# gildas-lormeau/zlib-streams-ts

Measured on AMD Instinct MI355X. Metric: uncompressed MB/s, deflate-raw L6, 4096x64KiB batch at 1/2/4/8 GPUs, higher is better.
Workload: dtype u8; 1 GPU; 4096 x 65536 B text-corpus streams split across the GPUs, deflate-raw level 6; global_streams=4096, streams_per_gpu=4096, stream_bytes=65536, level=6, format=deflate-raw, compressed_bytes=91855591, parallelism=dp1

## Files before the change

zlib-streams-ts_amd/csrc/capi.cpp:

```cpp
#include <hip/hip_runtime.h>
#include <stdint.h>
#include <stdio.h>
#include <string.h>

#include <algorithm>
#include <string>
#include <thread>
#include <vector>

#include "../../include/zs_gpu.h"
#include "zs_common.h"
#include "zs_kernels.h"
#include "zs_inflate.h"
#include "zs_split.h"
#include "zs_seg.h"
#include "zs_plan.h"
#include "zs_sweep_ring.h"
#include "zs_dict.h"


namespace {

thread_local std::string g_err;

// ... 958 lines not shown
  const zs_meta_layout ml(n);
  Batch b;
  const int r = upload_batch(c, st, ml, ml.bytes + (seeds ? 4ull * n : 0), {n, d_in, in_off, in_len, nullptr, nullptr, nullptr},
                             &b, [&](uint8_t* hm) { if (seeds) memcpy(hm + ml.bytes, seeds, 4ull * n); });
  if (r != ZS_OK) return r;
  MARK("start");
  zs_k_checksum<<<n, 64, 0, st>>>(b.in, b.in_off, b.in_len, d_check, kind,
                                  seeds ? (const uint32_t*)(c->meta.as<uint8_t>() + ml.bytes) : nullptr);
  MARK("checksum");
  HIPCHK(hipGetLastError());
  return ZS_OK;
}

extern "C" int zs_crc32_batch_device(zs_ctx* c, uint32_t n, const uint8_t* d_in, const uint64_t* in_off,
                                     const uint32_t* in_len, const uint32_t* seeds, uint32_t* d_check,
                                     void* hip_stream) {
  return checksum_batch(c, 2, n, d_in, in_off, in_len, seeds, d_check, hip_stream);
}
extern "C" int zs_adler32_batch_device(zs_ctx* c, uint32_t n, const uint8_t* d_in, const uint64_t* in_off,
                                       const uint32_t* in_len, const uint32_t* seeds, uint32_t* d_check,
                                       void* hip_stream) {
  return checksum_batch(c, 1, n, d_in, in_off, in_len, seeds, d_check, hip_stream);
}

static int checksum_host(zs_ctx* c, int kind, uint32_t n, const uint8_t* in, const uint64_t* in_off,
                         const uint32_t* in_len, const uint32_t* seeds, uint32_t* check) {
  if (!c) return fail(ZS_STREAM_ERROR, "null context");
  HIPCHK(hipSetDevice(c->device));
  if (n == 0) return ZS_OK;
  std::vector<uint64_t> doff;
  uint64_t total = 0;
  int r = stage_in(c, n, in, in_off, in_len, doff, total);
  if (r != ZS_OK) return r;
  HIPCHK(c->d_res.ensure(4ull * n + 16));
  r = checksum_batch(c, kind, n, c->d_in.as<uint8_t>(), doff.data(), in_len, seeds, c->d_res.as<uint32_t>(), nullptr);
  if (r != ZS_OK) return r;
  HIPCHK(hipMemcpyAsync(check, c->d_res.p, 4ull * n, hipMemcpyDeviceToHost, c->stream));
  HIPCHK(hipStreamSynchronize(c->stream));
  return ZS_OK;
}
extern "C" int zs_crc32_batch(zs_ctx* c, uint32_t n, const uint8_t* in, const uint64_t* in_off,
                              const uint32_t* in_len, const uint32_t* seeds, uint32_t* check) {
  return checksum_host(c, 2, n, in, in_off, in_len, seeds, check);
}
extern "C" int zs_adler32_batch(zs_ctx* c, uint32_t n, const uint8_t* in, const uint64_t* in_off,
                                const uint32_t* in_len, const uint32_t* seeds, uint32_t* check) {
  return checksum_host(c, 1, n, in, in_off, in_len, seeds, check);
}

namespace {
const char* kVocab =
    "the of and to in is that for it as was with be by on not he this are or his from at which but have an they you "
    "were her she there been one all we their has would when if so no will more can out said up what about its into "
    "them than only other new some could time these two may then do first any my now such like our over man me even "
    "most made after also did many before must through back years where much your way well down should because each "
    "just those people how too little state good very make world still own see men work long get here between both "
    "life being under never day same another know while last might us great old year off come since against go came "
    "right used take three";

struct XS {
  uint32_t s;
  explicit XS(uint32_t seed) : s(seed ? seed : 1) {}
  uint32_t operator()() {
    s ^= s << 13;
    s ^= s >> 17;
    s ^= s << 5;
    return s;
  }
};

void gen_text(uint32_t seed, uint8_t* out, uint32_t n, const std::vector<std::string>& V) {
  XS r(seed);
  uint32_t o = 0, w = 0;
  while (o < n) {
    const uint32_t a = r();
    const uint32_t idx = std::min(a % 144u, (a >> 12) % 144u);
    const std::string& word = V[idx];
    for (size_t i = 0; i < word.size() && o < n; i++) out[o++] = (uint8_t)word[i];
    if (o < n) out[o++] = (++w % 13 == 0) ? 10 : 32;
  }
}
}

extern "C" void zs_corpus(int kind, uint32_t first, uint32_t n_streams, uint32_t len, uint8_t* out, int threads) {
  std::vector<std::string> V;
  {
    std::string all(kVocab), cur;
    for (char ch : all) {
      if (ch == ' ') { V.push_back(cur); cur.clear(); }
      else cur.push_back(ch);
    }
    V.push_back(cur);
  }
  auto one = [&](uint32_t i) {
    const uint32_t seed = 0x9e3779b9u ^ (first + i);
    uint8_t* o = out + (size_t)i * len;
    if (kind == 2) {
      XS r(seed);
      for (uint32_t j = 0; j < len; j++) o[j] = (uint8_t)r();
      return;
    }
    gen_text(seed, o, len, V);
    if (kind == 1) {
      XS r(seed ^ 0x85ebca6bu);
      for (uint32_t k = 0; k + 8192 <= len; k += 8192)
        for (uint32_t j = 0; j < 1024; j++) o[k + 4096 + j] = (uint8_t)r();
    }
  };
  if (threads < 1) threads = 1;
  std::vector<std::thread> th;
  for (int t = 0; t < threads; t++)
    th.emplace_back([&, t] {
      for (uint32_t i = (uint32_t)t; i < n_streams; i += (uint32_t)threads) one(i);
    });
  for (auto& x : th) x.join();
}

extern "C" uint64_t zs_debug_fetch(zs_ctx* c, int what, uint32_t s, void* dst, uint64_t cap) {
  if (c && what >= 16 && what <= 21) {
    (void)hipSetDevice(c->device);
    (void)hipDeviceSynchronize();
    const Buf* b = what == 16 ? &c->gcnt : what == 17 ? &c->gblk : what == 18 ? &c->glanes : what == 19 ? &c->gmem
                   : what == 21 ? &c->gent : &c->gfound;
    const uint64_t bytes = std::min<uint64_t>(cap, b->cap);
    if (!b->p || !bytes || hipMemcpy(dst, b->p, bytes, hipMemcpyDeviceToHost) != hipSuccess) return 0;
    return bytes;
  }
  if (!c || !c->streams.p) return 0;
  (void)hipSetDevice(c->device);
  (void)hipStreamSynchronize(c->stream);
  (void)hipDeviceSynchronize();
  zs_stream st;
  if (hipMemcpy(&st, c->streams.as<zs_stream>() + s, sizeof st, hipMemcpyDeviceToHost) != hipSuccess) return 0;
  uint64_t pos_base = 0;
  uint32_t blk_base = 0, n = 0;
  const size_t nstreams = c->last_n;
  zs_meta_layout m2((uint32_t)nstreams);
  const uint8_t* hm = c->hmeta.data();
  pos_base = ((const uint64_t*)(hm + m2.pos_base))[s];
  blk_base = ((const uint32_t*)(hm + m2.blk_base))[s];
  n = ((const uint32_t*)(hm + m2.in_len))[s];
  if (s < c->dp.start.size()) n += c->dp.start[s];
  const void* src = nullptr;
  uint64_t bytes = 0;
  if ((what == 0 && 2ull * (pos_base + n) > c->prevd.cap) || (what == 1 && 8ull * (pos_base + n) > c->mres.cap)) return 0;
  switch (what) {
    case 0: src = c->prevd.as<uint16_t>() + pos_base; bytes = 2ull * n; break;
    case 1: src = c->mres.as<uint2>() + pos_base; bytes = 8ull * n; break;
    case 2: src = c->syms.as<uint32_t>() + pos_base + s; bytes = 4ull * st.nsym; break;
    case 3: src = c->blocks.as<zs_block>() + blk_base; bytes = sizeof(zs_block) * st.nblk; break;
    case 4: src = c->streams.as<zs_stream>() + s; bytes = sizeof(zs_stream); break;
    case 5: src = c->codes.as<uint32_t>() + (size_t)blk_base * (ZS_L_CODES + ZS_D_CODES); bytes = 4ull * (ZS_L_CODES + ZS_D_CODES) * st.nblk; break;
    case 6: src = c->hdr.as<uint32_t>() + (size_t)blk_base * ZS_HDR_WORDS; bytes = 4ull * ZS_HDR_WORDS * st.nblk; break;
    default: return 0;
  }
  bytes = std::min(bytes, cap);
  if (bytes && hipMemcpy(dst, src, bytes, hipMemcpyDeviceToHost) != hipSuccess) return 0;
  return bytes;
}

static const char* kInflateMsgs[ZS_MSG_COUNT] = {
    "",
    "incorrect header check",
    "unknown compression method",
    "invalid window size",
    "unknown header flags set",
    "header crc mismatch",
    "invalid block type",
    "invalid stored block lengths",
    "too many length or distance symbols",
    "too many length",
    "invalid code lengths set",
    "invalid bit length repeat",
    "invalid code -- missing end-of-block",
    "invalid literal/lengths set",
    "invalid distances set",
    "invalid literal/length code",
    "invalid distance code",
    "invalid distance too far back",
    "incorrect data check",
    "incorrect length check",
    "output capacity exceeded",
};

extern "C" const char* zs_inflate_message(int32_t i) { return (i >= 0 && i < ZS_MSG_COUNT) ? kInflateMsgs[i] : ""; }

__global__ void zs_k_inflate_finish(const zs_inflate_result* r, const zs_lane_res* lane, int32_t* status,
                                    int32_t* phase, int32_t* msg, uint32_t* out_len, uint32_t* consumed, int n,
                                    uint32_t* lane_count) {
  const int s = blockIdx.x * blockDim.x + threadIdx.x;
  if (s >= n) return;
  if (lane && lane[s].bail == 0) {
    atomicAdd(lane_count, 1u);
    status[s] = ZS_Z_STREAM_END;
    phase[s] = ZS_PHASE_NONE_;
    msg[s] = ZS_MSG_NONE;
    out_len[s] = lane[s].out_len;
    consumed[s] = lane[s].consumed;
    return;
  }
  status[s] = r[s].status;
  phase[s] = r[s].phase;
  msg[s] = r[s].msg;
  out_len[s] = r[s].out_len;
  consumed[s] = r[s].consumed;
}

__global__ void zs_k_inflate_check(const uint8_t* in, const uint64_t* in_off, const int32_t* status,
                                   const uint32_t* consumed, int wbits, uint32_t* out, int n) {
  const int s = blockIdx.x * blockDim.x + threadIdx.x;
  if (s >= n) return;
  uint32_t v = 0;
  if (status[s] == ZS_Z_STREAM_END && wbits > 0) {
    const uint8_t* t = in + in_off[s] + consumed[s] - (wbits == 31 ? 8 : 4);
    v = wbits == 31 ? (uint32_t)t[0] | (uint32_t)t[1] << 8 | (uint32_t)t[2] << 16 | (uint32_t)t[3] << 24
                    : (uint32_t)t[0] << 24 | (uint32_t)t[1] << 16 | (uint32_t)t[2] << 8 | (uint32_t)t[3];
  }
  out[s] = v;
}

static auto lane_kernel(int rt, bool refw) {
  return refw ? (rt == 2 ? zs_k_inflate_lane<2, true> : zs_k_inflate_lane<0, true>)
              : (rt == 2   ? zs_k_inflate_lane<2, false>
                 : rt == 1 ? zs_k_inflate_lane<1, false>
                           : zs_k_inflate_lane<0, false>);
}
static auto lane_kernel_dict(int rt) {
  return rt == 2 ? zs_k_inflate_lane<2, false, true> : rt == 1 ? zs_k_inflate_lane<1, false, true>
                                                               : zs_k_inflate_lane<0, false, true>;
}

static int seg_launch(zs_ctx* c, hipStream_t st, int wbits, const Batch& h, const Batch& b, zs_lane_res* lres) {
  const std::vector<uint32_t>& list = c->ip.seg;
  zs_seg_plan& p = c->gp;
  zs_plan_seg(c->o, wbits, list, h.in_len, h.out_cap, p);
  const uint32_t ng = (uint32_t)list.size(), nb = p.nb, nbig = (uint32_t)p.big.size();
  HIPCHK(c->glist.ensure(4ull * ng));
  HIPCHK(c->gspb.ensure(4ull * (ng + 1)));
  HIPCHK(c->gbig.ensure(4ull * nbig + 4));
  HIPCHK(c->gfound.ensure(8ull * ZS_SPLIT_MAX * nbig + 8));
  HIPCHK(c->gblk.ensure(sizeof(zs_seg_blk) * nb));
  HIPCHK(c->glanes.ensure(sizeof(zs_seg_lane) * ZS_SEG_LANES * nb));
  HIPCHK(c->gtab.ensure(sizeof(zcode) * ZS_SEG_TAB * nb));
  HIPCHK(c->gent.ensure(sizeof(zs_seg_ent) * ZS_SPLIT_MAX * ng));
  HIPCHK(c->gmem.ensure(sizeof(zs_seg_mem) * ng));
  HIPCHK(c->gpbase.ensure(4ull * (ng + 1)));
  HIPCHK(c->gplist.ensure(16ull * p.pbase[ng] + 16));
  HIPCHK(c->gsbase.ensure(8ull * (ng + 1)));
  HIPCHK(c->gscr.ensure(2ull * p.sbase[ng] + 64));
  HIPCHK(c->gcnt.ensure(16));
  HIPCHK(c->gspl.ensure(4ull * nb + 4));
  HIPCHK(c->gflist.ensure(4ull * ng));
  if (nbig) HIPCHK(c->gbigs.ensure(4ull * nbig));
  HIPCHK(hipMemcpyAsync(c->glist.p, list.data(), 4ull * ng, hipMemcpyHostToDevice, st));
  HIPCHK(hipMemcpyAsync(c->gspb.p, p.spb.data(), 4ull * (ng + 1), hipMemcpyHostToDevice, st));
  HIPCHK(hipMemcpyAsync(c->gpbase.p, p.pbase.data(), 4ull * (ng + 1), hipMemcpyHostToDevice, st));
  HIPCHK(hipMemcpyAsync(c->gsbase.p, p.sbase.data(), 8ull * (ng + 1), hipMemcpyHostToDevice, st));
  if (nbig) {
    HIPCHK(hipMemcpyAsync(c->gbigs.p, p.big_s.data(), 4ull * nbig, hipMemcpyHostToDevice, st));
    HIPCHK(hipMemcpyAsync(c->gbig.p, p.big.data(), 4ull * nbig, hipMemcpyHostToDevice, st));
  }
  HIPCHK(hipMemsetAsync(c->gmem.p, 0, sizeof(zs_seg_mem) * ng, st));
  HIPCHK(hipMemsetAsync(c->gent.p, 0, sizeof(zs_seg_ent) * ZS_SPLIT_MAX * ng, st));
  HIPCHK(hipMemsetAsync(c->gblk.p, 0xff, sizeof(zs_seg_blk) * nb, st));
  HIPCHK(hipMemsetAsync(c->gcnt.as<uint32_t>() + 2, 0, 8, st));
  if (!c->keep_counts) HIPCHK(hipMemsetAsync(c->gcnt.p, 0, 8, st));
  HIPCHK(hipEventRecord(c->fork, st));
  HIPCHK(hipStreamWaitEvent(c->side, c->fork, 0));
  hipStream_t sd = c->side;
  if (int r = mark(c, sd, "start")) return r;
  const uint32_t* gl = c->glist.as<uint32_t>();
  uint64_t* gf = c->gfound.as<uint64_t>();
  uint32_t* cnt = c->gcnt.as<uint32_t>();
  zs_seg_blk* gb = c->gblk.as<zs_seg_blk>();
  zs_seg_lane* gln = c->glanes.as<zs_seg_lane>();
  zcode* gt = c->gtab.as<zcode>();
  zs_seg_ent* ge = c->gent.as<zs_seg_ent>();
  zs_seg_mem* gm = c->gmem.as<zs_seg_mem>();
  const uint32_t* spl = c->gspl.as<uint32_t>();
  const uint64_t* sb = c->gsbase.as<uint64_t>();
  uint16_t* scr = c->gscr.as<uint16_t>();
  uint32_t* llen = c->llen.as<uint32_t>();
  if (nbig) {
    zs_k_split_find<<<nbig * ZS_SPLIT_MAX, 256, 0, sd>>>(b.in, b.in_off, b.in_len, c->gbigs.as<uint32_t>(), wbits, gf);
    if (int r = mark(c, sd, "seg_find")) return r;
  }
  auto walk = p.d64 ? (p.w2k ? zs_k_seg_walk<true, 2048u, false> : zs_k_seg_walk<true, 1024u, false>)
                    : (p.w2k ? zs_k_seg_walk<false, 2048u, true>
                             : p.large ? zs_k_seg_walk<false, 1024u, true> : zs_k_seg_walk<false, 1024u, false>);
  walk<<<p.nwalk, 64, 0, sd>>>(b.in, b.in_off, b.in_len, gl, ng, c->gbig.as<uint32_t>(), nbig, wbits, gf,
                               c->gspb.as<uint32_t>(), gb, gln, gt, ge, gm, cnt + 2, c->gspl.as<uint32_t>(), p.walk_bits,
                               p.split);
  if (int r = mark(c, sd, "seg_walk")) return r;
  zs_k_seg_plan<<<ng, 64, 0, sd>>>(b.in, b.in_off, b.in_len, b.out_cap, gl, ng, wbits, p.refw ? 1 : 0, gb, gln, ge, gm,
                                   c->gpbase.as<uint32_t>(), c->gplist.as<uint4>());
  if (int r = mark(c, sd, "seg_plan")) return r;
  auto decode = p.d64 ? zs_k_seg_decode<true, false> : p.refw ? zs_k_seg_decode<false, true> : zs_k_seg_decode<false, false>;
  decode<<<p.gdec, 64, 0, sd>>>(b.in, b.in_off, b.in_len, gl, cnt + 2, spl, gb, gln, gt, gm, sb, scr);
  if (int r = mark(c, sd, "seg_decode")) return r;
  const int rsm = p.rsmall ? 65536 : 32768;
  auto resolve = p.rsmall ? zs_k_seg_resolve<512u, 65536u> : zs_k_seg_resolve<256u, 32768u>;
  HIPCHK(hipFuncSetAttribute((const void*)resolve, hipFuncAttributeMaxDynamicSharedMemorySize, rsm));
  resolve<<<ng, p.rsmall ? 512u : 256u, rsm, sd>>>(gl, gm, c->gpbase.as<uint32_t>(), c->gplist.as<uint4>(), sb, scr, b.out,
                                             b.out_off, lres, llen, cnt + 1, cnt + 3, c->gflist.as<uint32_t>());
  if (int r = mark(c, sd, "seg_resolve")) return r;
  const size_t wsm = zs_inflate_wave_lds_bytes(p.d64);
// ... 292 lines not shown
```

zlib-streams-ts_amd/csrc/deflate_sweep.hip:

```cpp
#include <hip/hip_runtime.h>
#include "zs_common.h"
#include "zs_kernels.h"
#include "zs_sweep_ring.h"
#include "zs_sweep_long.h"
#include "zs_sweep_ends.h"
#include <type_traits>
#include <utility>

#define ZS_SW_WIN_WORDS ((ZS_SEG_WPOS + 258u + 20u + 3u) / 4u + 2u)
#define ZS_SW_RING 128u
#define ZS_SW_MW 320u
#ifndef ZS_SW_RUN_CAP
#define ZS_SW_RUN_CAP 16u
#endif

typedef __attribute__((address_space(3))) uint32_t zs_sw_lds_u32;
static __device__ __forceinline__ uint32_t sw_lds_addr(const void* p) {
  return (uint32_t)(uintptr_t)(const zs_sw_lds_u32*)p;
}

static __device__ __forceinline__ uint32_t sw_hash(uint32_t w) {
  return (((w & 0xffu) << 10) ^ (((w >> 8) & 0xffu) << 5) ^ ((w >> 16) & 0xffu)) & ZS_HASH_MASK;
}

#define ZS_BK_WPT (16384u / ZS_BK_THREADS)
#define ZS_BK_PPL (ZS_BK_THREADS / 64u)
#ifndef ZS_BK_PROF
#define ZS_BK_PROF 0
#endif
#if ZS_BK_PROF
__device__ unsigned long long zs_bk_stat[4];
extern "C" int zs_bucket_stats(unsigned long long* out) {
  return (int)hipMemcpyFromSymbol(out, HIP_SYMBOL(zs_bk_stat), sizeof(zs_bk_stat));
}
#define BK_MARK(i) do { if (threadIdx.x == 0) { const unsigned long long t_ = wall_clock64(); atomicAdd(&zs_bk_stat[i], t_ - bk_t); bk_t = t_; } } while (0)
#else
#define BK_MARK(i) do { } while (0)
#endif
#define ZS_BK_INFLIGHT 8
#define ZS_BK_CHUNK 2048u

template <bool ORD>
__global__ __launch_bounds__(ZS_BK_THREADS) void zs_k_bucket(const uint8_t* __restrict__ in,
                                                            const uint64_t* __restrict__ in_off,
                                                            const uint32_t* __restrict__ in_len,
                                                            const uint64_t* __restrict__ pos_base,
                                                            const zs_sweep_seg* __restrict__ segs,
                                                            uint16_t* __restrict__ members, uint2* __restrict__ mres) {
  __shared__ uint32_t cnt[16384];
  __shared__ uint32_t part[ZS_BK_THREADS];
  __shared__ uint32_t stg[ZS_BK_CHUNK / 4 + 2];
  __shared__ uint16_t q[2][ZS_BK_CHUNK];
  const zs_sweep_seg G = segs[blockIdx.x];
  const int s = (int)G.s;
  const uint32_t nrel = in_len[s] - G.base;
  const uint32_t tid = threadIdx.x;
  const uint8_t* src = in + in_off[s] + G.base;
  uint16_t* mem = members + G.mb;
  uint2* out = mres + pos_base[s] + G.base;
  const uint32_t m = nrel > 2 ? min(nrel - 2, G.ohi) : 0u;
  const uint32_t n = min(nrel, m + 2u);
  if (nrel - m <= 2u)
    for (uint32_t p = m + tid; p < nrel; p += ZS_BK_THREADS) out[p] = make_uint2(0, 0);
  if (m == 0) return;
  for (uint32_t i = tid; i < 16384 / 4; i += ZS_BK_THREADS) reinterpret_cast<uint4*>(cnt)[i] = make_uint4(0, 0, 0, 0);
  const bool aligned = ((uintptr_t)src & 3u) == 0;
#if ZS_BK_PROF
  unsigned long long bk_t = wall_clock64();
  if (threadIdx.x == 0) atomicAdd(&zs_bk_stat[3], 1ull);
#endif
  __syncthreads();
  {
    uint32_t w[5], nw[5];
    auto load5 = [&](uint32_t p0, uint32_t* x) __attribute__((always_inline)) {
#pragma unroll
      for (int k = 0; k < 5; k++) x[k] = zs_load_word(src, n, p0 + 16 * tid + 4 * k);
    };
    load5(0, nw);
    for (uint32_t p0 = 0; p0 < m; p0 += 16 * ZS_BK_THREADS) {
#pragma unroll
      for (int k = 0; k < 5; k++) w[k] = nw[k];
      if (p0 + 16 * ZS_BK_THREADS < m) load5(p0 + 16 * ZS_BK_THREADS, nw);
#pragma unroll
      for (uint32_t j = 0; j < 16; j++) {
        const uint32_t p = p0 + 16 * tid + j;
        const uint32_t h = sw_hash(__builtin_amdgcn_alignbyte(w[(j >> 2) + 1], w[j >> 2], j & 3u));
        if (p < m) atomicAdd(&cnt[h >> 1], 1u << (16u * (h & 1u)));
      }
    }
  }
  __syncthreads();
  BK_MARK(0);
  {
    uint32_t sum = 0;
    for (uint32_t j = 0; j < ZS_BK_WPT; j++) {
      const uint32_t w = cnt[ZS_BK_WPT * tid + ((j + tid) & (ZS_BK_WPT - 1u))];
      sum += (w & 0xffffu) + (w >> 16);
    }
    part[tid] = sum;
    __syncthreads();
    if (tid < 64) {
      uint32_t v[ZS_BK_PPL], t = 0;
#pragma unroll
      for (uint32_t j = 0; j < ZS_BK_PPL; j++) { v[j] = part[ZS_BK_PPL * tid + j]; t += v[j]; }
      uint32_t x = t;
#pragma unroll
      for (int d = 1; d < 64; d <<= 1) {
        const uint32_t y = __shfl_up(x, d, 64);
        if (tid >= (uint32_t)d) x += y;
      }
      uint32_t run = x - t;
#pragma unroll
      for (uint32_t j = 0; j < ZS_BK_PPL; j++) { part[ZS_BK_PPL * tid + j] = run; run += v[j]; }
    }
    __syncthreads();
    uint32_t run = part[tid];
    for (uint32_t j = 0; j < ZS_BK_WPT; j++) {
      const uint32_t w = cnt[ZS_BK_WPT * tid + j];
      const uint32_t lo = w & 0xffffu;
      cnt[ZS_BK_WPT * tid + j] = run | ((run + lo) << 16);
      run += lo + (w >> 16);
    }
  }
  __syncthreads();
  BK_MARK(1);
  const uint32_t wave = tid >> 6, lane = tid & 63u;
  constexpr uint32_t CW = ZS_BK_CHUNK / 4 / 64;
  uint32_t nxt[CW + 1];
  auto fetch = [&](uint32_t c0) {
#pragma unroll
    for (uint32_t i = 0; i <= CW; i++) {
      const uint32_t w = 64 * i + lane;
      const uint32_t at = c0 + 4 * w;
      uint32_t v = 0;
      if (w < ZS_BK_CHUNK / 4 + 2) {
        if (aligned && at + 4 <= n) v = *(const uint32_t*)(src + at);
        else
          for (uint32_t k = 0; k < 4; k++)
            if (at + k < n) v |= (uint32_t)src[at + k] << (8 * k);
      }
      nxt[i] = v;
    }
  };
  if (wave == 0) fetch(0);
  const uint32_t nch = (m + ZS_BK_CHUNK - 1) / ZS_BK_CHUNK;
  for (uint32_t c = 0; c <= nch; c++) {
    const uint32_t c0 = c * ZS_BK_CHUNK;
    if (wave == 0 && c < nch) {
      __builtin_amdgcn_s_waitcnt(0xc07f);
      __builtin_amdgcn_wave_barrier();
#pragma unroll
      for (uint32_t i = 0; i <= CW; i++)
        if (64 * i + lane < ZS_BK_CHUNK / 4 + 2) stg[64 * i + lane] = nxt[i];
      __builtin_amdgcn_s_waitcnt(0xc07f);
      __builtin_amdgcn_wave_barrier();
      if (c0 + ZS_BK_CHUNK < m) fetch(c0 + ZS_BK_CHUNK);
      const uint32_t c1 = min(m, c0 + ZS_BK_CHUNK);
      uint16_t* const qc = q[c & 1u];
      for (uint32_t g0 = c0; g0 < c1; g0 += 64 * ZS_BK_INFLIGHT) {
        uint32_t a[ZS_BK_INFLIGHT], v[ZS_BK_INFLIGHT], sh[ZS_BK_INFLIGHT], e[ZS_BK_INFLIGHT], hh[ZS_BK_INFLIGHT];
#pragma unroll
        for (int j = 0; j < ZS_BK_INFLIGHT; j++) {
          const uint32_t p = g0 + 64 * j + lane;
          const uint32_t o = p - c0;
          const uint32_t h = sw_hash(__builtin_amdgcn_alignbyte(stg[(o >> 2) + 1], stg[o >> 2], o & 3u));
          hh[j] = h;
          sh[j] = 16u * (h & 1u);
          a[j] = sw_lds_addr(&cnt[h >> 1]);
          v[j] = p < c1 ? 1u << sh[j] : 0u;
        }
        if (!ORD) {
#pragma unroll
          for (int j = 0; j < ZS_BK_INFLIGHT; j++) {
            const uint32_t p = g0 + 64 * j + lane;
            const uint32_t h = hh[j];
            const uint64_t mm = zs_wave_match(h, p < c1);
            const uint32_t rank = (uint32_t)__builtin_popcountll(mm & ((1ull << lane) - 1ull));
            const uint32_t lead = mm ? (uint32_t)__builtin_ctzll(mm) : lane;
            uint32_t old = 0;
            if (p < c1 && lead == lane)
              old = atomicAdd(&cnt[h >> 1], (uint32_t)__builtin_popcountll(mm) << sh[j]);
            old = (uint32_t)__builtin_amdgcn_ds_bpermute((int)(lead * 4u), (int)old);
            e[j] = old + (rank << sh[j]);
          }
        } else {
        asm volatile(
            "ds_add_rtn_u32 %0, %8, %16\n\t"
            "ds_add_rtn_u32 %1, %9, %17\n\t"
            "ds_add_rtn_u32 %2, %10, %18\n\t"
            "ds_add_rtn_u32 %3, %11, %19\n\t"
            "ds_add_rtn_u32 %4, %12, %20\n\t"
            "ds_add_rtn_u32 %5, %13, %21\n\t"
            "ds_add_rtn_u32 %6, %14, %22\n\t"
            "ds_add_rtn_u32 %7, %15, %23\n\t"
            "s_waitcnt lgkmcnt(0)"
            : "=&v"(e[0]), "=&v"(e[1]), "=&v"(e[2]), "=&v"(e[3]), "=&v"(e[4]), "=&v"(e[5]), "=&v"(e[6]), "=&v"(e[7])
            : "v"(a[0]), "v"(a[1]), "v"(a[2]), "v"(a[3]), "v"(a[4]), "v"(a[5]), "v"(a[6]), "v"(a[7]), "v"(v[0]),
              "v"(v[1]), "v"(v[2]), "v"(v[3]), "v"(v[4]), "v"(v[5]), "v"(v[6]), "v"(v[7])
            : "memory");
        }
#pragma unroll
        for (int j = 0; j < ZS_BK_INFLIGHT; j++) {
          const uint32_t p = g0 + 64 * j + lane;
          if (p < c1) qc[p - c0] = (uint16_t)(e[j] >> sh[j]);
        }
      }
    } else if (wave != 0 && c > 0) {
      const uint32_t b0 = c0 - ZS_BK_CHUNK, cnt1 = min(m, c0) - b0;
      const uint16_t* const qp = q[(c - 1) & 1u];
      for (uint32_t o = tid - 64u; o < cnt1; o += ZS_BK_THREADS - 64u) mem[qp[o]] = (uint16_t)(b0 + o);
    }
    __syncthreads();
  }
  BK_MARK(2);
}
template __global__ void zs_k_bucket<true>(const uint8_t*, const uint64_t*, const uint32_t*, const uint64_t*,
                                           const zs_sweep_seg*, uint16_t*, uint2*);
template __global__ void zs_k_bucket<false>(const uint8_t*, const uint64_t*, const uint32_t*, const uint64_t*,
                                            const zs_sweep_seg*, uint16_t*, uint2*);

static __device__ __forceinline__ uint32_t sw_word(const uint32_t* win, uint32_t off) {
  const uint32_t i = off >> 2;
  return __builtin_amdgcn_alignbyte(win[i + 1], win[i], off & 3u);
}

static __device__ __forceinline__ uint32_t sw_extend(const uint32_t* win, uint32_t p, uint32_t q, uint32_t maxc,
                                                     uint32_t from) {
  uint32_t k = from;
  while (k < maxc) {
    const uint32_t y = sw_word(win, q + k) ^ sw_word(win, p + k);
    if (y) { k += (uint32_t)(__builtin_ctz(y) >> 3); break; }
    k += 4;
  }
  return k < maxc ? k : maxc;
}

static __device__ __forceinline__ uint32_t max3(uint32_t a, uint32_t b, uint32_t c) {
  return max(max(a, b), c);
}

static __device__ __forceinline__ uint32_t sw_x7(uint32_t w) {
  const uint32_t b0 = w & 0xffu, b1 = (w >> 8) & 0xffu;
  return ((b0 >> 5) & 3u) | ((b1 & 7u) << 2) | (((b1 >> 5) & 3u) << 5);
}
template <bool A7>
struct SwSig;
template <>
struct SwSig<false> {
  static constexpr uint32_t LONG = 88u;
  static constexpr uint32_t THR0 = 23u;
  static constexpr uint32_t EXT = 11u;
  uint32_t a, b, c;
  static __device__ __forceinline__ uint4 rec(const uint32_t* win, uint32_t q, uint32_t w0) {
    return make_uint4(w0, sw_word(win, q + 4), sw_word(win, q + 8) & 0x00ffffffu, 0u);
  }
  __device__ __forceinline__ uint32_t mbits(uint32_t x, uint32_t y, uint32_t z) const {
    uint32_t f0, f1, f2;
    asm("v_ffbl_b32 %0, %1" : "=v"(f0) : "v"(x ^ a));
    asm("v_ffbl_b32 %0, %1\n\tv_add_u32_e64 %0, %0, 32 clamp" : "=&v"(f1) : "v"(y ^ b));
    asm("v_ffbl_b32 %0, %1\n\tv_add_u32_e32 %0, 64, %0" : "=&v"(f2) : "v"(z ^ c));
    return min(min(f0, f1), f2);
  }
  template <uint32_t U>
  __device__ __forceinline__ uint32_t step(uint32_t x, uint32_t y, uint32_t z) const {
    return (mbits(x, y, z) & ~7u) | (7u - U);
  }
  template <uint32_t U>
  __device__ __forceinline__ uint32_t step(uint32_t x, uint32_t y, uint32_t z, uint64_t lm) const {
    uint32_t r;
    asm("v_cndmask_b32_e64 %0, 0, %1, %2" : "=v"(r) : "v"(step<U>(x, y, z)), "s"(lm));
    return r;
  }
  static __device__ __forceinline__ uint32_t len(uint32_t sigma) { return sigma; }
};
template <>
struct SwSig<true> {
  static constexpr uint32_t LONG = 64u;
  static constexpr uint32_t THR0 = 7u;
  static constexpr uint32_t EXT = 10u;
  uint32_t a, b;
  static __device__ __forceinline__ uint4 rec(const uint32_t* win, uint32_t q, uint32_t w0) {
    return make_uint4(sw_x7(w0) | (sw_word(win, q + 3) << 8), sw_word(win, q + 6), sw_word(win, q + EXT), 0u);
  }
  __device__ __forceinline__ uint32_t mbits(uint32_t x, uint32_t y, uint32_t) const {
    uint32_t f0, f1;
    asm("v_ffbl_b32 %0, %1" : "=v"(f0) : "v"(x ^ a));
    asm("v_ffbl_b32 %0, %1\n\tv_add_u32_e64 %0, %0, 32 clamp" : "=&v"(f1) : "v"(y ^ b));
    return min(min(f0, f1), 64u);
  }
  template <uint32_t U>
  __device__ __forceinline__ uint32_t step(uint32_t x, uint32_t y, uint32_t) const {
    uint32_t t;
    asm("v_xor_b32_e32 %0, %0, %3\n\t"
        "v_xor_b32_e32 %1, %2, %4\n\t"
        "v_ffbl_b32 %0, %0\n\t"
        "v_ffbl_b32 %1, %1\n\t"
        "v_add_u32_e64 %1, %1, 32 clamp\n\t"
        "v_min3_u32 %0, %0, %1, 64\n\t"
        "v_and_or_b32 %0, %0, -8, %5"
        : "+v"(x), "=v"(t)
        : "v"(y), "v"(a), "v"(b), "n"(7u - U));
    return x;
  }
  template <uint32_t U>
  __device__ __forceinline__ uint32_t step(uint32_t x, uint32_t y, uint32_t, uint64_t lm) const {
    uint32_t t;
    asm("v_xor_b32_e32 %0, %0, %3\n\t"
        "v_xor_b32_e32 %1, %2, %4\n\t"
        "v_ffbl_b32 %0, %0\n\t"
        "v_ffbl_b32 %1, %1\n\t"
        "v_add_u32_e64 %1, %1, 32 clamp\n\t"
        "v_min3_u32 %0, %0, %1, 64\n\t"
        "v_and_or_b32 %0, %0, -8, %5\n\t"
        "v_cndmask_b32_e64 %0, 0, %0, %6"
        : "+v"(x), "=v"(t)
        : "v"(y), "v"(a), "v"(b), "n"(7u - U), "s"(lm));
    return x;
  }
  static __device__ __forceinline__ uint32_t len(uint32_t sigma) { return sigma ? sigma + 2u : 2u; }
};

struct SwRing {
  uint2 ab[2 * ZS_SW_RING];
  uint32_t c[2 * ZS_SW_RING];
  uint32_t key[2 * ZS_SW_RING];
  __device__ __forceinline__ void put(int b, uint32_t lane, uint4 r) {
    const uint32_t i = (uint32_t)(64 * b + (int)lane) & (ZS_SW_RING - 1);
    ab[i] = make_uint2(r.x, r.y);
    ab[i + ZS_SW_RING] = make_uint2(r.x, r.y);
    c[i] = r.z;
    c[i + ZS_SW_RING] = r.z;
    key[i] = r.w;
    key[i + ZS_SW_RING] = r.w;
  }
  static __device__ __forceinline__ uint32_t base(int c, uint32_t s, uint32_t lane) {
    return ((uint32_t)(64 * (c - (int)s - 1) + (int)lane) & (ZS_SW_RING - 1)) + 64u * s + 64u;
  }
};
struct SwRingP {
  uint2 ab[ZS_SWR_SLOTS + ZS_SWR_MIRROR];
  uint32_t c[ZS_SWR_SLOTS + ZS_SWR_MIRROR];
  uint32_t key[ZS_SWR_SLOTS + ZS_SWR_MIRROR];
  __device__ __forceinline__ void put(int b, uint32_t lane, uint4 r) {
    const uint32_t i = zs_swr_block_slot(b) + lane;
    ab[i] = make_uint2(r.x, r.y);
    c[i] = r.z;
    key[i] = r.w;
    if (zs_swr_mirrored(b)) {
      ab[i + ZS_SWR_SLOTS] = make_uint2(r.x, r.y);
      c[i + ZS_SWR_SLOTS] = r.z;
      key[i + ZS_SWR_SLOTS] = r.w;
    }
  }
  static __device__ __forceinline__ uint32_t base(int c, uint32_t s, uint32_t lane) { return zs_swr_base(c, s) + lane; }
  __device__ __forceinline__ uint32_t pos(int c, uint32_t lane, uint32_t t) const {
    return key[zs_swr_member_slot(c, lane, t)] & 0xffffu;
  }
};

#ifndef ZS_SW_PROF
#define ZS_SW_PROF 0
#endif
#if ZS_SW_PROF
__device__ unsigned long long zs_sw_stat[8];
#define SW_STAT(i, v) do { if ((threadIdx.x & 63u) == __builtin_ctzll(__builtin_amdgcn_read_exec())) atomicAdd(&zs_sw_stat[i], (unsigned long long)(v)); } while (0)
// ... 577 lines not shown
```

zlib-streams-ts_amd/zsamd/__init__.py:

```python
from __future__ import annotations

import ctypes
import os
from typing import List, Optional, Sequence, Tuple

_HERE = os.path.dirname(os.path.abspath(__file__))
LIB_PATH = os.environ.get("ZS_LIB") or os.path.join(os.path.dirname(_HERE), "libzsgpu.so")

Z_OK, Z_STREAM_END, Z_NEED_DICT = 0, 1, 2
Z_STREAM_ERROR, Z_DATA_ERROR, Z_MEM_ERROR, Z_BUF_ERROR = -2, -3, -4, -5
PHASE_NONE, PHASE_INIT, PHASE_PROCESS, PHASE_FINISH = 0, 1, 2, 3
Z_DEFAULT_STRATEGY, Z_FILTERED, Z_HUFFMAN_ONLY, Z_RLE, Z_FIXED = 0, 1, 2, 3, 4

def compress_wbits(fmt: str) -> int:
    return 31 if fmt == "gzip" else (-15 if fmt == "deflate-raw" else 15)


def decompress_wbits(fmt: str) -> int:
    if fmt == "gzip":
        return 31
    if fmt == "deflate-raw":
        return -15
    if fmt == "deflate64-raw":
        return -16
# ... 67 lines not shown
    L = ctypes.CDLL(LIB_PATH)
    L.zs_ctx_create.argtypes = [ctypes.c_int, ctypes.POINTER(_P)]
    L.zs_ctx_destroy.argtypes = [_P]
    L.zs_last_error.restype = ctypes.c_char_p
    L.zs_version.restype = ctypes.c_char_p
    L.zs_deflate_bound.restype = ctypes.c_uint64
    L.zs_deflate_bound.argtypes = [ctypes.c_uint64, ctypes.c_int]
    L.zs_deflate_batch_device.argtypes = [_P, ctypes.c_int, ctypes.c_int, ctypes.c_uint32, _P, _U64P, _U32P, _P, _U64P,
                                          _U32P, _P, _P, _P]
    L.zs_deflate_batch.argtypes = [_P, ctypes.c_int, ctypes.c_int, ctypes.c_uint32, ctypes.c_char_p, _U64P, _U32P,
                                   _P, _U64P, _U32P, _I32P, _U32P]
    L.zs_deflate_batch_ex.argtypes = L.zs_deflate_batch.argtypes + [_U32P]
    L.zs_deflate_batch_device_ex.argtypes = [_P, ctypes.c_int, ctypes.c_int, ctypes.c_uint32, _P, _U64P, _U32P, _P,
                                             _U64P, _U32P, _P, _P, _P, _P]
    _inf_host = [ctypes.c_int, ctypes.c_uint32, ctypes.c_char_p, _U64P, _U32P]
    _inf_res = [_I32P, _I32P, _I32P, _U32P, _U32P, _U32P]
    L.zs_inflate_batch_ex.argtypes = [_P] + _inf_host + [_P, _U64P, _U32P] + _inf_res
    L.zs_inflate_batch_auto.argtypes = [_P] + _inf_host + [ctypes.POINTER(_P), _U64P] + _inf_res
    _dict = [ctypes.c_char_p, _U64P, _U32P]
    if hasattr(L, "zs_inflate_batch_dict"):
        L.zs_inflate_batch_dict.argtypes = L.zs_inflate_batch_ex.argtypes + _dict
        L.zs_inflate_batch_dict_auto.argtypes = L.zs_inflate_batch_auto.argtypes + _dict
        L.zs_inflate_batch_dict_device.argtypes = [_P, ctypes.c_int, ctypes.c_uint32, _P, _U64P, _U32P, _P, _U64P,
                                                   _U32P, _P, _P, _P, _P, _P, _P, _P, _P, _U64P, _U32P]
    if hasattr(L, "zs_deflate_batch_dict"):
        L.zs_deflate_bound_dict.restype = ctypes.c_uint64
        L.zs_deflate_bound_dict.argtypes = [ctypes.c_uint64, ctypes.c_int, ctypes.c_uint64]
        L.zs_deflate_batch_dict.argtypes = L.zs_deflate_batch_ex.argtypes + _dict
        L.zs_deflate_batch_dict_device.argtypes = L.zs_deflate_batch_device_ex.argtypes + [_P, _U64P, _U32P]
    if hasattr(L, "zs_deflate_batch_strategy"):
        _with = lambda a: a[:2] + [ctypes.c_int] + a[2:]
        L.zs_deflate_batch_strategy.argtypes = _with(L.zs_deflate_batch_ex.argtypes)
        L.zs_deflate_batch_strategy_device.argtypes = _with(L.zs_deflate_batch_device_ex.argtypes)
        L.zs_pool_deflate_batch_strategy.argtypes = _with(L.zs_deflate_batch_ex.argtypes)
    if hasattr(L, "zs_deflate_batch_params"):
        _withm = lambda a: a[:3] + [ctypes.c_int] + a[3:]
        L.zs_deflate_batch_params.argtypes = _withm(L.zs_deflate_batch_ex.argtypes)
        L.zs_deflate_batch_params_device.argtypes = _withm(L.zs_deflate_batch_device_ex.argtypes)
        L.zs_pool_deflate_batch_params.argtypes = _withm(L.zs_deflate_batch_ex.argtypes)
        L.zs_deflate_bound_params.restype = ctypes.c_uint64
        L.zs_deflate_bound_params.argtypes = [ctypes.c_uint64, ctypes.c_int, ctypes.c_int, ctypes.c_int]
    L.zs_free.argtypes = [_P]
    L.zs_pool_create.argtypes = [ctypes.c_uint64, ctypes.POINTER(_P)]
    L.zs_pool_create_list.argtypes = [ctypes.POINTER(ctypes.c_int), ctypes.c_int, ctypes.POINTER(_P)]
    L.zs_pool_destroy.argtypes = [_P]
    L.zs_pool_size.argtypes = [_P]
    L.zs_pool_device.argtypes = [_P, ctypes.c_int]
    L.zs_pool_deflate_batch.argtypes = L.zs_deflate_batch_ex.argtypes
    L.zs_pool_inflate_batch.argtypes = L.zs_inflate_batch_ex.argtypes
    L.zs_pool_inflate_batch_auto.argtypes = L.zs_inflate_batch_auto.argtypes
    if hasattr(L, "zs_pool_inflate_batch_dict"):
        L.zs_pool_inflate_batch_dict.argtypes = L.zs_inflate_batch_dict.argtypes
        L.zs_pool_inflate_batch_dict_auto.argtypes = L.zs_inflate_batch_dict_auto.argtypes
    if hasattr(L, "zs_pool_deflate_batch_dict"):
        L.zs_pool_deflate_batch_dict.argtypes = L.zs_deflate_batch_dict.argtypes
    if hasattr(L, "zs_inflate_batch"):
        L.zs_inflate_batch.argtypes = [_P, ctypes.c_int, ctypes.c_uint32, ctypes.c_char_p, _U64P, _U32P, _P, _U64P,
                                       _U32P, _I32P, _I32P, _I32P, _U32P, _U32P]
        L.zs_inflate_batch_device.argtypes = [_P, ctypes.c_int, ctypes.c_uint32, _P, _U64P, _U32P, _P, _U64P, _U32P,
                                              _P, _P, _P, _P, _P, _P]
        L.zs_inflate_message.restype = ctypes.c_char_p
        L.zs_inflate_message.argtypes = [ctypes.c_int32]
    L.zs_crc32_batch_device.argtypes = [_P, ctypes.c_uint32, _P, _U64P, _U32P, _U32P, _P, _P]
    L.zs_adler32_batch_device.argtypes = [_P, ctypes.c_uint32, _P, _U64P, _U32P, _U32P, _P, _P]
    L.zs_crc32_batch.argtypes = [_P, ctypes.c_uint32, ctypes.c_char_p, _U64P, _U32P, _U32P, _U32P]
    L.zs_adler32_batch.argtypes = [_P, ctypes.c_uint32, ctypes.c_char_p, _U64P, _U32P, _U32P, _U32P]
    L.zs_last_batch_ms.restype = ctypes.c_double
    L.zs_last_batch_ms.argtypes = [_P]
    L.zs_last_inflate_lane_count.restype = ctypes.c_uint32
    L.zs_last_inflate_lane_count.argtypes = [_P]
    L.zs_last_inflate_seg_count.restype = ctypes.c_uint32
    L.zs_last_inflate_seg_count.argtypes = [_P]
    L.zs_last_phase_ms.restype = ctypes.c_double
    L.zs_last_phase_ms.argtypes = [_P, ctypes.c_char_p]
    L.zs_set_timing.argtypes = [_P, ctypes.c_int]
    L.zs_corpus.argtypes = [ctypes.c_int, ctypes.c_uint32, ctypes.c_uint32, ctypes.c_uint32, _P, ctypes.c_int]
    L.zs_selftest.argtypes = [_P, _U64P]
    L.zs_set_option.argtypes = [_P, ctypes.c_char_p, ctypes.c_int]
    L.zs_debug_fetch.restype = ctypes.c_uint64
    L.zs_debug_fetch.argtypes = [_P, ctypes.c_int, ctypes.c_uint32, _P, ctypes.c_uint64]
    _lib = L
    return L


def build_id() -> str:
    import hashlib

    h = hashlib.sha256()
    csrc = os.path.join(os.path.dirname(_HERE), "csrc")
    files = sorted(f for f in os.listdir(csrc) if f.endswith((".hip", ".cpp", ".h")) or f == "Makefile")
    for f in files + ["../../include/zs_gpu.h"]:
        h.update(f.encode() + b"\0")
        with open(os.path.join(csrc, f), "rb") as fh:
            h.update(fh.read())
    return h.hexdigest()[:16]


def _arr(ctype, values):
    a = (ctype * max(1, len(values)))(*values)
    return a


def deflate_bound(n: int, fmt: str = "deflate-raw", dict_len: int = 0) -> int:
    if dict_len:
        return int(lib().zs_deflate_bound_dict(n, compress_wbits(fmt), dict_len))
    return int(lib().zs_deflate_bound(n, compress_wbits(fmt)))


def deflate_capacity(n: int, fmt: str = "deflate-raw", dict_len: int = 0) -> int:
    return (deflate_bound(n, fmt, dict_len) + 3) & ~3


class Engine:

    def __init__(self, device: int = 0):
        L = lib()
        ctx = _P()
        r = L.zs_ctx_create(device, ctypes.byref(ctx))
        if r != 0:
            raise ZsUnavailable("zs_ctx_create(%d) failed: %s" % (device, L.zs_last_error().decode()))
        self._L, self._ctx, self.device = L, ctx, device

    def selftest(self) -> int:
        v = ctypes.c_uint64(0)
        r = self._L.zs_selftest(self._ctx, ctypes.byref(v))
        if r != 0:
            raise ZsError("zs_selftest failed: %s" % self._L.zs_last_error().decode())
        return int(v.value)

    def close(self):
        if getattr(self, "_ctx", None):
            self._L.zs_ctx_destroy(self._ctx)
            self._ctx = None

    def __del__(self):
        try:
            self.close()
        except Exception:
            pass

    @property
    def handle(self):
        return self._ctx

    def set_option(self, name: str, value: int):
        if self._L.zs_set_option(self._ctx, name.encode(), int(value)) != 0:
            raise ZsError(self._L.zs_last_error().decode())

    def debug_fetch(self, what: int, stream: int, nbytes: int) -> bytes:
        buf = ctypes.create_string_buffer(max(1, nbytes))
        k = self._L.zs_debug_fetch(self._ctx, what, stream, buf, nbytes)
        return buf.raw[:k]

    def set_timing(self, on: bool):
        self._L.zs_set_timing(self._ctx, 1 if on else 0)

    def last_lane_count(self) -> int:
        return self._L.zs_last_inflate_lane_count(self._ctx)

    def last_seg_count(self) -> int:
        return self._L.zs_last_inflate_seg_count(self._ctx)

    def last_ms(self, phase: Optional[str] = None) -> float:
        if phase is None:
            return self._L.zs_last_batch_ms(self._ctx)
        return self._L.zs_last_phase_ms(self._ctx, phase.encode())

    def _check(self, r: int, what: str):
        if r != 0:
            msg = self._L.zs_last_error().decode()
            if r == Z_STREAM_ERROR:
                raise ZsError("init failed: %d" % r, r, PHASE_INIT, msg)
            raise ZsUnavailable("%s failed (%d): %s" % (what, r, msg))

    def compress_batch_raw(self, inputs: Sequence[bytes], fmt: str = "deflate-raw", level: int = -1, zdict=None,
                           strategy: int = 0, window_bits=None, mem_level=8) -> List[Tuple[int, bytes]]:
        return [(st, b) for st, b, _ in self.compress_batch_detailed(inputs, fmt, level, zdict, strategy, window_bits,
                                                                     mem_level)]

    def compress_batch_detailed(self, inputs: Sequence[bytes], fmt: str = "deflate-raw", level: int = -1, zdict=None,
                                strategy: int = 0, window_bits=None, mem_level=8) -> List[Tuple[int, bytes, int]]:
        compress_strategy(strategy, zdict)
        code = compress_params(fmt, window_bits, mem_level, zdict, strategy)
        if not _params_default(window_bits, mem_level):
            return _deflate_host(self._L, self._L.zs_deflate_batch_params, self._ctx, inputs, fmt, level, self._check,
                                 params=(code, mem_level))
        if compress_strategy(strategy, zdict):
            return _deflate_host(self._L, self._L.zs_deflate_batch_strategy, self._ctx, inputs, fmt, level,
                                 self._check, strategy=strategy)
        if zdict is not None:
            return _deflate_host(self._L, self._L.zs_deflate_batch_dict, self._ctx, inputs, fmt, level, self._check,
                                 _dict_layout(zdict, len(inputs)))
        return _deflate_host(self._L, self._L.zs_deflate_batch_ex, self._ctx, inputs, fmt, level, self._check)

    def compress_batch(self, inputs: Sequence[bytes], fmt: str = "deflate-raw", level: int = -1, zdict=None,
                       strategy: int = 0, window_bits=None, mem_level=8) -> List[bytes]:
        return _ok_or_raise_c(self.compress_batch_raw(inputs, fmt, level, zdict, strategy, window_bits, mem_level))

    def decompress_batch_raw(self, inputs: Sequence[bytes], fmt: str = "deflate-raw",
                             out_caps: Optional[Sequence[int]] = None, zdict=None):
        return [r[:5] for r in self.decompress_batch_detailed(inputs, fmt, out_caps, zdict)]

    def decompress_batch_detailed(self, inputs: Sequence[bytes], fmt: str = "deflate-raw",
                                  out_caps: Optional[Sequence[int]] = None, zdict=None):
        L = self._L
        if zdict is not None:
            d = _dict_layout(zdict, len(inputs))
            if out_caps is None:
                return _inflate_host_auto(L, L.zs_inflate_batch_dict_auto, self._ctx, inputs, fmt, self._check, d)
            return _inflate_host(L, L.zs_inflate_batch_dict, self._ctx, inputs, fmt, out_caps, self._check, d)
        if out_caps is None:
            return _inflate_host_auto(L, L.zs_inflate_batch_auto, self._ctx, inputs, fmt, self._check)
        return _inflate_host(L, L.zs_inflate_batch_ex, self._ctx, inputs, fmt, out_caps, self._check)

    def decompress_batch(self, inputs: Sequence[bytes], fmt: str = "deflate-raw",
                         out_caps: Optional[Sequence[int]] = None, zdict=None) -> List[bytes]:
        return _ok_or_raise_d(self.decompress_batch_raw(inputs, fmt, out_caps, zdict))

    def compress_device(self, level: int, fmt: str, n: int, d_in: int, in_off, in_len, d_out: int, out_off, out_cap,
                        d_status: int, d_out_len: int, hip_stream: int = 0, d_check: int = 0, d_dict: int = 0,
                        dict_off=None, dict_len=None, strategy: int = 0, window_bits=None, mem_level=8):
        compress_strategy(strategy, dict_off)
        code = compress_params(fmt, window_bits, mem_level, dict_off, strategy)
        if not _params_default(window_bits, mem_level):
            r = self._L.zs_deflate_batch_params_device(self._ctx, compress_level(level), code, mem_level, n, _P(d_in),
                                                       in_off, in_len, _P(d_out), out_off, out_cap, _P(d_status),
                                                       _P(d_out_len), _P(d_check) if d_check else None,
                                                       _P(hip_stream) if hip_stream else None)
            self._check(r, "zs_deflate_batch_params_device")
            return
        if compress_strategy(strategy, dict_off):
            r = self._L.zs_deflate_batch_strategy_device(self._ctx, compress_level(level), strategy,
                                                         compress_wbits(fmt), n, _P(d_in), in_off, in_len, _P(d_out),
                                                         out_off, out_cap, _P(d_status), _P(d_out_len),
                                                         _P(d_check) if d_check else None,
                                                         _P(hip_stream) if hip_stream else None)
            self._check(r, "zs_deflate_batch_strategy_device")
            return
        if dict_off is not None:
            r = self._L.zs_deflate_batch_dict_device(self._ctx, compress_level(level), compress_wbits(fmt), n,
                                                     _P(d_in), in_off, in_len, _P(d_out), out_off, out_cap,
                                                     _P(d_status), _P(d_out_len), _P(d_check) if d_check else None,
                                                     _P(hip_stream) if hip_stream else None,
                                                     _P(d_dict) if d_dict else None, dict_off, dict_len)
            self._check(r, "zs_deflate_batch_dict_device")
            return
        r = self._L.zs_deflate_batch_device_ex(self._ctx, compress_level(level), compress_wbits(fmt), n, _P(d_in),
                                               in_off, in_len, _P(d_out), out_off, out_cap, _P(d_status),
                                               _P(d_out_len), _P(d_check) if d_check else None,
                                               _P(hip_stream) if hip_stream else None)
        self._check(r, "zs_deflate_batch_device")

    def decompress_device(self, fmt: str, n: int, d_in: int, in_off, in_len, d_out: int, out_off, out_cap,
                          d_status: int, d_phase: int, d_msg: int, d_out_len: int, d_consumed: int,
                          hip_stream: int = 0, d_dict: int = 0, dict_off=None, dict_len=None, d_check: int = 0):
        if dict_off is not None:
            r = self._L.zs_inflate_batch_dict_device(self._ctx, decompress_wbits(fmt), n, _P(d_in), in_off, in_len,
                                                     _P(d_out), out_off, out_cap, _P(d_status), _P(d_phase),
                                                     _P(d_msg), _P(d_out_len), _P(d_consumed),
                                                     _P(d_check) if d_check else None,
                                                     _P(hip_stream) if hip_stream else None,
                                                     _P(d_dict) if d_dict else None, dict_off, dict_len)
            self._check(r, "zs_inflate_batch_dict_device")
            return
        r = self._L.zs_inflate_batch_device(self._ctx, decompress_wbits(fmt), n, _P(d_in), in_off, in_len, _P(d_out),
                                            out_off, out_cap, _P(d_status), _P(d_phase), _P(d_msg), _P(d_out_len),
                                            _P(d_consumed), _P(hip_stream) if hip_stream else None)
        self._check(r, "zs_inflate_batch_device")

    def compress_host(self, level: int, fmt: str, n: int, h_in: int, in_off, in_len, h_out: int, out_off, out_cap,
                      status, out_len, strategy: int = 0, window_bits=None, mem_level=8):
        compress_strategy(strategy)
        code = compress_params(fmt, window_bits, mem_level, None, strategy)
        if not _params_default(window_bits, mem_level):
            r = self._L.zs_deflate_batch_params(self._ctx, level, code, mem_level, n,
                                                ctypes.cast(h_in, ctypes.c_char_p), in_off, in_len, _P(h_out), out_off,
                                                out_cap, status, out_len, None)
            self._check(r, "zs_deflate_batch_params")
            return
        if compress_strategy(strategy):
            r = self._L.zs_deflate_batch_strategy(self._ctx, level, strategy, compress_wbits(fmt), n,
                                                  ctypes.cast(h_in, ctypes.c_char_p), in_off, in_len, _P(h_out),
                                                  out_off, out_cap, status, out_len, None)
            self._check(r, "zs_deflate_batch_strategy")
            return
        r = self._L.zs_deflate_batch(self._ctx, level, compress_wbits(fmt), n, ctypes.cast(h_in, ctypes.c_char_p),
                                     in_off, in_len, _P(h_out), out_off, out_cap, status, out_len)
        self._check(r, "zs_deflate_batch")

    def decompress_host(self, fmt: str, n: int, h_in: int, in_off, in_len, h_out: int, out_off, out_cap, status,
                        phase, msg, out_len, consumed):
        r = self._L.zs_inflate_batch(self._ctx, decompress_wbits(fmt), n, ctypes.cast(h_in, ctypes.c_char_p), in_off,
                                     in_len, _P(h_out), out_off, out_cap, status, phase, msg, out_len, consumed)
        self._check(r, "zs_inflate_batch")

    def checksum_device(self, kind: str, n: int, d_in: int, in_off, in_len, d_check: int, hip_stream: int = 0,
                        seeds=None):
        fn = self._L.zs_crc32_batch_device if kind == "crc32" else self._L.zs_adler32_batch_device
        r = fn(self._ctx, n, _P(d_in), in_off, in_len, seeds, _P(d_check), _P(hip_stream) if hip_stream else None)
        self._check(r, "checksum")

    def checksum(self, kind: str, bufs: Sequence[bytes], seeds: Optional[Sequence[int]] = None) -> List[int]:
        n = len(bufs)
        if n == 0:
            return []
        offs, lens, o = [], [], 0
# ... 277 lines not shown
```

Before: 22750 MB/s.

## Sort bucket scatter stores by destination slot to coalesce member writes

```diff
diff --git a/zlib-streams-ts_amd/csrc/capi.cpp b/zlib-streams-ts_amd/csrc/capi.cpp
--- a/zlib-streams-ts_amd/csrc/capi.cpp
+++ b/zlib-streams-ts_amd/csrc/capi.cpp
@@ -1134,6 +1134,16 @@
     case 4: src = c->streams.as<zs_stream>() + s; bytes = sizeof(zs_stream); break;
     case 5: src = c->codes.as<uint32_t>() + (size_t)blk_base * (ZS_L_CODES + ZS_D_CODES); bytes = 4ull * (ZS_L_CODES + ZS_D_CODES) * st.nblk; break;
     case 6: src = c->hdr.as<uint32_t>() + (size_t)blk_base * ZS_HDR_WORDS; bytes = 4ull * ZS_HDR_WORDS * st.nblk; break;
+    case 7: {
+      const zs_deflate_plan& p = c->dp;
+      if (p.match != ZS_MATCH_SWEEP || (size_t)s + 1 >= p.win0.size()) return 0;
+      const zs_sweep_seg& g = p.segs[p.win0[s]];
+      const uint32_t m = n > 2 ? std::min(n - 2, g.ohi) : 0u;
+      if (2ull * (g.mb + m) > c->prevd.cap) return 0;
+      src = c->prevd.as<uint16_t>() + g.mb;
+      bytes = 2ull * m;
+      break;
+    }
     default: return 0;
   }
   bytes = std::min(bytes, cap);
diff --git a/zlib-streams-ts_amd/csrc/deflate_sweep.hip b/zlib-streams-ts_amd/csrc/deflate_sweep.hip
--- a/zlib-streams-ts_amd/csrc/deflate_sweep.hip
+++ b/zlib-streams-ts_amd/csrc/deflate_sweep.hip
@@ -39,6 +39,13 @@
 #endif
 #define ZS_BK_INFLIGHT 8
 #define ZS_BK_CHUNK 2048u
+#define ZS_BK_KEYS 256u
+#define ZS_BK_HELPERS (ZS_BK_THREADS - 64u)
+#define ZS_BK_EPT ((ZS_BK_CHUNK + ZS_BK_HELPERS - 1u) / ZS_BK_HELPERS)
+
+static __device__ __forceinline__ void bk_lds_barrier() {
+  asm volatile("s_waitcnt lgkmcnt(0)\n\ts_barrier" ::: "memory");
+}
 
 template <bool ORD>
 __global__ __launch_bounds__(ZS_BK_THREADS) void zs_k_bucket(const uint8_t* __restrict__ in,
@@ -48,7 +55,8 @@
                                                             const zs_sweep_seg* __restrict__ segs,
                                                             uint16_t* __restrict__ members, uint2* __restrict__ mres) {
   __shared__ uint32_t cnt[16384];
-  __shared__ uint32_t part[ZS_BK_THREADS];
+  __shared__ uint32_t part[ZS_BK_KEYS + ZS_BK_CHUNK / 2];
+  static_assert(ZS_BK_KEYS + ZS_BK_CHUNK / 2 >= ZS_BK_THREADS, "part[] holds the scan's partial sums");
   __shared__ uint32_t stg[ZS_BK_CHUNK / 4 + 2];
   __shared__ uint16_t q[2][ZS_BK_CHUNK];
   const zs_sweep_seg G = segs[blockIdx.x];
@@ -125,6 +133,13 @@
   __syncthreads();
   BK_MARK(1);
   const uint32_t wave = tid >> 6, lane = tid & 63u;
+  constexpr uint32_t PH = ZS_BK_CHUNK / (64 * ZS_BK_INFLIGHT);
+  static_assert(PH == 4, "a chunk is four steps: count, scan, place, store");
+  uint32_t* const kc = part;
+  uint16_t* const srt = reinterpret_cast<uint16_t*>(part + ZS_BK_KEYS);
+  if (tid < ZS_BK_KEYS) kc[tid] = 0;
+  uint32_t sl[ZS_BK_EPT];
+  const uint32_t ht = tid - 64u;
   constexpr uint32_t CW = ZS_BK_CHUNK / 4 / 64;
   uint32_t nxt[CW + 1];
   auto fetch = [&](uint32_t c0) {
@@ -146,18 +161,25 @@
   const uint32_t nch = (m + ZS_BK_CHUNK - 1) / ZS_BK_CHUNK;
   for (uint32_t c = 0; c <= nch; c++) {
     const uint32_t c0 = c * ZS_BK_CHUNK;
+    const uint32_t c1 = min(m, c0 + ZS_BK_CHUNK);
+    const uint32_t b0 = c0 - ZS_BK_CHUNK, cnt1 = min(m, c0) - b0;
+    const uint16_t* const qp = q[(c - 1) & 1u];
+#pragma unroll
+    for (uint32_t ph = 0; ph < PH; ph++) {
+    const uint32_t g0 = c0 + 64 * ZS_BK_INFLIGHT * ph;
     if (wave == 0 && c < nch) {
-      __builtin_amdgcn_s_waitcnt(0xc07f);
-      __builtin_amdgcn_wave_barrier();
-#pragma unroll
-      for (uint32_t i = 0; i <= CW; i++)
-        if (64 * i + lane < ZS_BK_CHUNK / 4 + 2) stg[64 * i + lane] = nxt[i];
-      __builtin_amdgcn_s_waitcnt(0xc07f);
-      __builtin_amdgcn_wave_barrier();
-      if (c0 + ZS_BK_CHUNK < m) fetch(c0 + ZS_BK_CHUNK);
-      const uint32_t c1 = min(m, c0 + ZS_BK_CHUNK);
+      if (ph == 0) {
+        __builtin_amdgcn_s_waitcnt(0xc07f);
+        __builtin_amdgcn_wave_barrier();
+#pragma unroll
+        for (uint32_t i = 0; i <= CW; i++)
+          if (64 * i + lane < ZS_BK_CHUNK / 4 + 2) stg[64 * i + lane] = nxt[i];
+        __builtin_amdgcn_s_waitcnt(0xc07f);
+        __builtin_amdgcn_wave_barrier();
+        if (c0 + ZS_BK_CHUNK < m) fetch(c0 + ZS_BK_CHUNK);
+      }
       uint16_t* const qc = q[c & 1u];
-      for (uint32_t g0 = c0; g0 < c1; g0 += 64 * ZS_BK_INFLIGHT) {
+      if (g0 < c1) {
         uint32_t a[ZS_BK_INFLIGHT], v[ZS_BK_INFLIGHT], sh[ZS_BK_INFLIGHT], e[ZS_BK_INFLIGHT], hh[ZS_BK_INFLIGHT];
 #pragma unroll
         for (int j = 0; j < ZS_BK_INFLIGHT; j++) {
@@ -206,11 +228,45 @@
         }
       }
     } else if (wave != 0 && c > 0) {
-      const uint32_t b0 = c0 - ZS_BK_CHUNK, cnt1 = min(m, c0) - b0;
-      const uint16_t* const qp = q[(c - 1) & 1u];
-      for (uint32_t o = tid - 64u; o < cnt1; o += ZS_BK_THREADS - 64u) mem[qp[o]] = (uint16_t)(b0 + o);
-    }
-    __syncthreads();
+      if (ph == 0) {
+#pragma unroll
+        for (uint32_t k = 0; k < ZS_BK_EPT; k++) {
+          const uint32_t o = ht + ZS_BK_HELPERS * k;
+          sl[k] = o < cnt1 ? (uint32_t)qp[o] : 0u;
+          if (o < cnt1) atomicAdd(&kc[sl[k] >> 8], 1u);
+        }
+      } else if (ph == 1) {
+        if (wave == 1) {
+          constexpr uint32_t KPL = ZS_BK_KEYS / 64u;
+          uint32_t v[KPL], t = 0;
+#pragma unroll
+          for (uint32_t j = 0; j < KPL; j++) { v[j] = kc[KPL * lane + j]; t += v[j]; }
+          uint32_t x = t;
+#pragma unroll
+          for (int d = 1; d < 64; d <<= 1) {
+            const uint32_t y = __shfl_up(x, d, 64);
+            if (lane >= (uint32_t)d) x += y;
+          }
+          uint32_t run = x - t;
+#pragma unroll
+          for (uint32_t j = 0; j < KPL; j++) { kc[KPL * lane + j] = run; run += v[j]; }
+        }
+      } else if (ph == 2) {
+#pragma unroll
+        for (uint32_t k = 0; k < ZS_BK_EPT; k++) {
+          const uint32_t o = ht + ZS_BK_HELPERS * k;
+          if (o < cnt1) srt[atomicAdd(&kc[sl[k] >> 8], 1u)] = (uint16_t)o;
+        }
+      } else {
+        for (uint32_t i = ht; i < cnt1; i += ZS_BK_HELPERS) {
+          const uint32_t o = srt[i];
+          mem[qp[o]] = (uint16_t)(b0 + o);
+        }
+        if (ht < ZS_BK_KEYS) kc[ht] = 0;
+      }
+    }
+    bk_lds_barrier();
+    }
   }
   BK_MARK(2);
 }
diff --git a/zlib-streams-ts_amd/zsamd/__init__.py b/zlib-streams-ts_amd/zsamd/__init__.py
--- a/zlib-streams-ts_amd/zsamd/__init__.py
+++ b/zlib-streams-ts_amd/zsamd/__init__.py
@@ -243,6 +243,9 @@
         k = self._L.zs_debug_fetch(self._ctx, what, stream, buf, nbytes)
         return buf.raw[:k]
 
+    def bucket_members(self, stream: int) -> bytes:
+        return self.debug_fetch(7, stream, 2 * 65535)
+
     def set_timing(self, on: bool):
         self._L.zs_set_timing(self._ctx, 1 if on else 0)
 
```

Measured after the change: 23490 MB/s (median of 6 runs). 3.3% higher.
